# mconati/armour-dev

Measured on AMD Instinct MI355X. Metric: planning iterations/sec (7-DOF, 100 t-steps, 20 obs), higher is better.
Workload: dtype f64; 1 GPU; Kinova Gen3 7-DOF, T=100, O=20 box obstacles, 3 concurrent planner(s) x 1308 worlds/GPU/step; obstacles=20, worlds_per_gpu=3924, planners_per_gpu=3, worlds_per_planner=1308, parallelism=world-sharded x1, RCCL all_gather of per-world records

## Files before the change

armour-dev_amd/armour_amd/__init__.py:

```python
from __future__ import annotations

import ctypes
import os

import numpy as np

from .robots import KINOVA
from .worlds import csv_world, example_world, make_world, straight_line_waypoint

_HERE = os.path.dirname(os.path.abspath(__file__))
LIB_PATH = os.environ.get("ARMOUR_LIB") or os.path.join(_HERE, "libarmour_hip.so")
NF = 7
_LIB = None
_dp = ctypes.POINTER(ctypes.c_double)


ARMOUR_E_ARG, ARMOUR_E_HIP, ARMOUR_E_CAPACITY, ARMOUR_E_STATE, ARMOUR_E_INTERNAL = -1, -2, -3, -4, -5


class ArmourError(RuntimeError):
    pass


class Config(ctypes.Structure):
    _fields_ = [("robot", ctypes.c_int), ("num_time_steps", ctypes.c_int), ("max_obstacles", ctypes.c_int),
                ("max_worlds", ctypes.c_int), ("device", ctypes.c_int), ("max_iter", ctypes.c_int)]


class World(ctypes.Structure):
    _fields_ = [("q0", ctypes.c_double * NF), ("qd0", ctypes.c_double * NF), ("qdd0", ctypes.c_double * NF),
                ("q_des", ctypes.c_double * NF), ("num_obstacles", ctypes.c_int), ("obstacles", _dp)]


_WORLD_DTYPE = np.dtype({"names": ["q0", "qd0", "qdd0", "q_des", "num_obstacles", "obstacles"],
                         "formats": [(np.float64, NF)] * 4 + [np.int32, np.uintp],
                         "offsets": [World.q0.offset, World.qd0.offset, World.qdd0.offset, World.q_des.offset,
                                     World.num_obstacles.offset, World.obstacles.offset],
                         "itemsize": ctypes.sizeof(World)})


class ArmtdWorld(ctypes.Structure):
    _fields_ = [("q0", ctypes.c_double * NF), ("qd0", ctypes.c_double * NF), ("q_des", ctypes.c_double * NF),
                ("jrs_tables", _dp), ("k_range", ctypes.c_double * NF), ("num_obstacles", ctypes.c_int),
                ("obstacles", _dp)]


class Result(ctypes.Structure):
    _fields_ = [("k_opt", ctypes.c_double * NF), ("feasible", ctypes.c_int), ("solver_status", ctypes.c_int),
                ("iterations", ctypes.c_int), ("evaluations", ctypes.c_int), ("cost", ctypes.c_double),
                ("kkt_error", ctypes.c_double), ("error", ctypes.c_int)]


class Timing(ctypes.Structure):
    _fields_ = [("reach_ms", ctypes.c_double), ("nlp_ms", ctypes.c_double), ("total_ms", ctypes.c_double),
                ("reach_kernel_ms", ctypes.c_double), ("reach_bytes", ctypes.c_double)]

    def as_dict(self):
        return {name: getattr(self, name) for name, _ in self._fields_}


class PlanOutput(ctypes.Structure):
    _fields_ = [("result", Result), ("timing", Timing), ("constraints", _dp), ("joint_bounds", _dp),
                ("link_centers", _dp), ("link_generators", _dp), ("torque_radius", _dp)]


def lib():
    global _LIB
    if _LIB is None:
        if not os.path.exists(LIB_PATH):
            raise ArmourError(f"HIP planner library not built: {LIB_PATH} (run __graft_entry__.build())")
        L = ctypes.CDLL(LIB_PATH)
        L.armour_create.restype = ctypes.c_void_p
        L.armour_create.argtypes = [ctypes.POINTER(Config)]
        L.armour_create_robot.restype = ctypes.c_void_p
        L.armour_create_robot.argtypes = [ctypes.POINTER(Config), ctypes.c_void_p]
        L.armour_robot_builtin.argtypes = [ctypes.c_int, ctypes.c_void_p]
        L.armour_device_compute_units.argtypes = [ctypes.c_int]
        L.armour_copy_bandwidth.restype = ctypes.c_double
        L.armour_copy_bandwidth.argtypes = [ctypes.c_int, ctypes.c_size_t, ctypes.c_int]
        L.armour_destroy.argtypes = [ctypes.c_void_p]
        L.armour_last_error.restype = ctypes.c_char_p
        L.armour_num_constraints.argtypes = [ctypes.c_void_p, ctypes.c_int]
        L.armour_num_joints.argtypes = [ctypes.c_void_p]
        L.armour_create_armtd.restype = ctypes.c_void_p
        L.armour_create_armtd.argtypes = [ctypes.POINTER(Config)]
        L.armour_plan_armtd_batch.argtypes = [ctypes.c_void_p, ctypes.c_int, ctypes.POINTER(ArmtdWorld),
                                              ctypes.POINTER(Result), ctypes.POINTER(Timing)]
        L.armour_reach_armtd_batch.argtypes = [ctypes.c_void_p, ctypes.c_int, ctypes.POINTER(ArmtdWorld),
                                               ctypes.POINTER(Timing)]
        L.armour_plan_batch.argtypes = [ctypes.c_void_p, ctypes.c_int, ctypes.POINTER(World), ctypes.POINTER(Result),
                                        ctypes.POINTER(Timing)]
        L.armour_reach_batch.argtypes = [ctypes.c_void_p, ctypes.c_int, ctypes.POINTER(World), ctypes.POINTER(Timing)]
        for name, args in (("armour_plan_batch_mixed", L.armour_plan_batch.argtypes),
                           ("armour_reach_batch_mixed", L.armour_reach_batch.argtypes),
                           ("armour_world_num_obstacles", [ctypes.c_void_p, ctypes.c_int]),
                           ("armour_eval_candidates", [ctypes.c_void_p, ctypes.c_int, _dp, _dp, _dp,
                                                       ctypes.POINTER(ctypes.c_int), ctypes.POINTER(ctypes.c_int)])):
            if hasattr(L, name):
                getattr(L, name).argtypes = args
        L.armour_plan.argtypes = [ctypes.c_void_p, ctypes.POINTER(World), ctypes.POINTER(PlanOutput)]
        L.armour_eval_constraints.argtypes = [ctypes.c_void_p, ctypes.c_int, _dp, _dp, _dp]
        L.armour_get_reach_program.argtypes = [ctypes.c_void_p, ctypes.POINTER(ctypes.c_int), ctypes.c_int]
        L.armour_get_monomial_counts.argtypes = [ctypes.c_void_p, ctypes.c_int, ctypes.POINTER(ctypes.c_int),
                                                 ctypes.POINTER(ctypes.c_int)]
        L.armour_get_reach_occupancy.argtypes = [ctypes.c_void_p, ctypes.POINTER(ctypes.c_longlong),
                                                 ctypes.POINTER(ctypes.c_longlong), ctypes.c_int]
        L.armour_get_joint_bounds.argtypes = [ctypes.c_void_p, _dp]
        L.armour_get_plane_cache_stats.argtypes = [ctypes.c_void_p, ctypes.POINTER(ctypes.c_longlong), ctypes.c_int]
        L.armour_get_reach_span.argtypes = [ctypes.c_void_p, _dp]
        L.armour_get_reach_dump.argtypes = [ctypes.c_void_p, _dp, ctypes.c_int]
        L.armour_get_reach_profile.argtypes = [ctypes.c_void_p, ctypes.POINTER(ctypes.c_ulonglong), ctypes.c_int]
        for name in ("armour_get_constraints", "armour_get_link_centers", "armour_get_link_generators",
                     "armour_get_torque_radius"):
            getattr(L, name).argtypes = [ctypes.c_void_p, ctypes.c_int, _dp]
        if hasattr(L, "armour_sq_selfcheck"):
            L.armour_sq_selfcheck.argtypes = [ctypes.c_int, ctypes.c_double, ctypes.c_longlong, _dp, ctypes.c_longlong,
                                              _dp, ctypes.POINTER(ctypes.c_int), ctypes.POINTER(ctypes.c_longlong)]
        _LIB = L
    return _LIB


ABI_SYMBOLS = ["armour_copy_bandwidth", "armour_create", "armour_create_robot", "armour_robot_builtin", "armour_device_compute_units", "armour_destroy", "armour_last_error", "armour_num_constraints",
               "armour_plan_batch", "armour_reach_batch", "armour_eval_constraints", "armour_get_constraints",
               "armour_get_link_centers", "armour_get_link_generators", "armour_get_torque_radius",
               "armour_num_joints", "armour_get_joint_bounds", "armour_get_reach_program", "armour_get_reach_profile",
               "armour_get_reach_dump", "armour_get_reach_occupancy", "armour_get_monomial_counts",
               "armour_create_armtd", "armour_plan_armtd_batch", "armour_reach_armtd_batch",
               "armour_get_plane_cache_stats", "armour_plan", "armour_get_reach_span",
               "armour_plan_batch_mixed", "armour_reach_batch_mixed", "armour_world_num_obstacles",
               "armour_eval_candidates", "armour_sq_selfcheck"]


def default_batch(T: int, device: int = 0, waves: int = 2) -> int:
    n = lib().armour_device_compute_units(device)
    _check(min(0, n))
    return max(1, (waves * n * 64) // T)


def copy_bandwidth(device: int = 0, nbytes: int = 2 << 30, reps: int = 10) -> float:
    v = lib().armour_copy_bandwidth(device, nbytes, reps)
    if v < 0:
        raise ArmourError(f"armour_copy_bandwidth: {lib().armour_last_error().decode()}")
    return v


def sq_selfcheck(thr: float, half_width: int, values=None, device: int = 0):
    v = np.ascontiguousarray(values if values is not None else np.zeros(0), dtype=np.float64)
    s, ok, bad = ctypes.c_double(0), ctypes.c_int(0), ctypes.c_longlong(0)
    _check(lib().armour_sq_selfcheck(device, float(thr), int(half_width), _ptr(v) if v.size else None, v.size,
                                     ctypes.byref(s), ctypes.byref(ok), ctypes.byref(bad)))
    return s.value, bool(ok.value), int(bad.value)


def _check(rc):
    if rc != 0:
        raise ArmourError(f"armour error {rc}: {lib().armour_last_error().decode()}")


def _ptr(a):
    return a.ctypes.data_as(_dp) if a is not None else None


def candidates_array(x, W):
    x = np.asarray(x, dtype=np.float64)
    if x.ndim == 2 and x.shape[1] == NF and x.shape[0] >= 1:
        if W < 1:
            raise ValueError("eval_candidates: x of shape [N, 7] needs a batch (reach or plan first)")
        x = np.broadcast_to(x, (W,) + x.shape)
    if x.ndim != 3 or x.shape[2] != NF or x.shape[0] < 1 or x.shape[1] < 1 or (W >= 1 and x.shape[0] != W):
        raise ValueError(f"eval_candidates: x must have shape [W, N, {NF}] or [N, {NF}] (W = {W}), got {x.shape}")
    if not np.all(np.isfinite(x)):
        raise ValueError("eval_candidates: x holds a non-finite value")
    if np.abs(x).max() > 1.0:
        raise ValueError("eval_candidates: every candidate must lie in [-1, 1]")
    return np.ascontiguousarray(x)


class Planner:

    def __init__(self, T=100, max_obstacles=20, max_worlds=1, device=0, max_iter=0, robot=None, _armtd=False):
        cfg = Config(0, T, max_obstacles, max_worlds, device, max_iter)
        if _armtd:
            self.h = lib().armour_create_armtd(ctypes.byref(cfg))
        elif robot is None:
            self.h = lib().armour_create(ctypes.byref(cfg))
        else:
            from .robot_tables import to_struct
            self._robot = to_struct(robot)
            self.h = lib().armour_create_robot(ctypes.byref(cfg), ctypes.byref(self._robot))
        if not self.h:
            raise ArmourError(f"armour_create failed: {lib().armour_last_error().decode()}")
        self.T = T
        self.NJ = lib().armour_num_joints(self.h)
        self.max_worlds = max_worlds
        self._keep = []
        self.O = 0
        self._W = 0

    def close(self):
        if getattr(self, "h", None) and _LIB is not None:
            _LIB.armour_destroy(self.h)
        self.h = None

    def __del__(self):
        self.close()

    def num_constraints(self, O):
        return lib().armour_num_constraints(self.h, O)

    def _worlds(self, worlds):
        n = len(worlds)
        arr = (World * n)()
        view = np.frombuffer(arr, dtype=_WORLD_DTYPE)
# ... 89 lines not shown
        J = np.zeros((m, NF)) if jac else None
        _check(lib().armour_eval_constraints(self.h, w, _ptr(x), _ptr(g), _ptr(J)))
        return (g, J) if jac else g

    def eval_candidates(self, x, num_worlds=None):
        x = candidates_array(x, self._W if num_worlds is None else int(num_worlds))
        Wx, N = x.shape[:2]
        cost = np.zeros((Wx, N))
        viol = np.zeros((Wx, N, 3))
        feas = np.zeros((Wx, N), dtype=np.int32)
        best = np.zeros(Wx, dtype=np.int32)
        ip = ctypes.POINTER(ctypes.c_int)
        _check(lib().armour_eval_candidates(self.h, N, _ptr(x), _ptr(cost), _ptr(viol), feas.ctypes.data_as(ip),
                                            best.ctypes.data_as(ip)))
        return dict(cost=cost, violation=viol, feasible=feas.astype(bool), best=best)

    def constraints(self, w):
        g = np.zeros(self._m(w))
        _check(lib().armour_get_constraints(self.h, w, _ptr(g)))
        return g

    def link_centers(self, w):
        c = np.zeros((self.T, self.NJ, 3))
        _check(lib().armour_get_link_centers(self.h, w, _ptr(c)))
        return c

    def link_generators(self, w):
        g = np.zeros((self.T, self.NJ, 3, 6))
        _check(lib().armour_get_link_generators(self.h, w, _ptr(g)))
        return g

    def joint_bounds(self):
        b = np.zeros(28)
        _check(lib().armour_get_joint_bounds(self.h, _ptr(b)))
        return b

    def reach_program(self):
        n = lib().armour_get_reach_program(self.h, None, 0)
        codes = (ctypes.c_int * n)()
        lib().armour_get_reach_program(self.h, codes, n)
        return np.array(codes[:])

    def reach_dump(self):
        n = lib().armour_get_reach_dump(self.h, None, 0)
        if n < 0:
            _check(n)
        d = np.zeros((n, 8))
        _check(min(0, lib().armour_get_reach_dump(self.h, _ptr(d), n)))
        return d

    def reach_profile(self):
        n = lib().armour_get_reach_profile(self.h, None, 0)
        if n < 0:
            _check(n)
        buf = (ctypes.c_ulonglong * (2 * n + 16))()
        _check(min(0, lib().armour_get_reach_profile(self.h, buf, n + 8)))
        a = np.array(buf[:], dtype=np.uint64)
        return a[:2 * n].reshape(n, 2), a[2 * n:]

    def monomial_counts(self, w):
        lk = np.zeros((self.T, self.NJ), dtype=np.int32)
        tq = np.zeros((self.T, NF), dtype=np.int32)
        _check(lib().armour_get_monomial_counts(self.h, w, lk.ctypes.data_as(ctypes.POINTER(ctypes.c_int)),
                                                tq.ctypes.data_as(ctypes.POINTER(ctypes.c_int))))
        return lk, tq

    OCCUPANCY = ("arena_hashes", "arena_rows", "operator_terms", "link_monomials", "torque_monomials",
                 "worlds_retried", "worlds_failed")

    def occupancy(self):
        n = len(self.OCCUPANCY)
        used = (ctypes.c_longlong * n)()
        caps = (ctypes.c_longlong * n)()
        rc = lib().armour_get_reach_occupancy(self.h, used, caps, n)
        _check(min(0, rc))
        return {k: (int(used[i]), int(caps[i])) for i, k in enumerate(self.OCCUPANCY)}

    def reach_span_ms(self):
        v = ctypes.c_double()
        _check(lib().armour_get_reach_span(self.h, ctypes.byref(v)))
        return v.value

    def plane_cache_stats(self):
        keys = ("planes_kept", "pairs", "blocks_cached", "blocks", "max_per_pair", "pool_records", "box_misses")
        out = (ctypes.c_longlong * len(keys))()
        _check(min(0, lib().armour_get_plane_cache_stats(self.h, out, len(keys))))
        return {k: int(out[i]) for i, k in enumerate(keys)}

    def torque_radius(self, w):
        r = np.zeros((self.T, NF))
        _check(lib().armour_get_torque_radius(self.h, w, _ptr(r)))
        return r


class ArmtdPlanner(Planner):

    def __init__(self, T=100, max_obstacles=20, max_worlds=1, device=0, max_iter=0):
        super().__init__(T=T, max_obstacles=max_obstacles, max_worlds=max_worlds, device=device, max_iter=max_iter,
                         _armtd=True)

    def _worlds(self, worlds):
        n = len(worlds)
        arr = (ArmtdWorld * n)()
        keep = []
        for k, (q0, qd0, q_des, tab, kr, obs) in enumerate(worlds):
            a = arr[k]
            a.q0[:] = [float(v) for v in q0]
            a.qd0[:] = [float(v) for v in qd0]
            a.q_des[:] = [float(v) for v in q_des]
            a.k_range[:] = [float(v) for v in kr]
            t = np.ascontiguousarray(np.asarray(tab, dtype=np.float64).reshape(NF, 6, self.T))
            o = np.ascontiguousarray(np.asarray(obs, dtype=np.float64).reshape(-1, 12))
            keep += [t, o]
            a.jrs_tables = _ptr(t)
            a.num_obstacles = o.shape[0]
            a.obstacles = _ptr(o) if o.shape[0] else None
        self._keep = keep
        self.O = arr[0].num_obstacles if n else 0
        self._W = n
        return arr

    def _plan_call(self, *a):
        return lib().armour_plan_armtd_batch(*a)

    def _reach_call(self, *a):
        return lib().armour_reach_armtd_batch(*a)


__all__ = ["ArmtdPlanner", "Planner", "ArmourError", "ARMOUR_E_CAPACITY", "ARMOUR_E_INTERNAL", "copy_bandwidth", "default_batch", "make_world", "example_world", "csv_world", "straight_line_waypoint", "KINOVA", "LIB_PATH", "ABI_SYMBOLS", "candidates_array"]
```

armour-dev_amd/csrc/nlp.h:

```cpp
#pragma once
#include "reach.h"

namespace armour {

constexpr int EVAL_THREADS = 256;
constexpr int ROW_THREADS = 256;
constexpr int MAX_FILTER = 64;
constexpr int KA = 56;
constexpr int KA2 = 8;

struct IpmOpts {
    double tol = 1e-4;
    int max_iter = 100;
    double mu0 = 0.1;
    double kappa_eps = 10.0;
    double kappa_mu = 0.2;
    double theta_mu = 1.5;
    double tau_min = 0.99;
    double bound_push = 1e-2;
    double eta = 1e-4;
    int max_ls = 10;
    double kappa_sigma = 1e10;
    double s_max = 100.0;
    double inf_bound = 1e19;
// ... 5 lines not shown
};

struct WorldState {
    double x[NF], xt[NF], dx[NF];
    double H[NF * NF];
    double mu, alpha, ap, ad, theta0, phi0, Dphi, theta_max, theta_min, kkt;
    double sw_dphi, sw_theta;
    double wa_old_a[NF], wa_old_b[NF];
    double filt_theta[MAX_FILTER], filt_phi[MAX_FILTER];
    int nfilt;
    int cur;
    int status;
    int searching;
    int accepted_ok;
    int ftype;
    int first_update, nfail, iter, nevals, ls;
    int spec_k;
    int free_mode, nref;
    double kkt_ref[4];
    int nresto, rstall, rpend;
    double rphi;
};
constexpr int WS_RESTO = 6;
constexpr int WS_RESTART = 7;

struct NlpDev {
    int W, T, NJ, O, m, R, nblk, chunk;
    int armtd, nt;
    const double* krange;
    int diag;
    const RobotParams* rp;
    IpmOpts opt;
    const double* q0;
    const double* qd0;
    const double* qdd0;
    const double* qdes;
    const double* obs;
    ReachOut ro;
    double *L, *U;
    double* g;
    double* J;
    double* jn;
    double* jd;
    long njn, njd;
    double* f;
    double* grad;
    double* link_c;
    long lcs;
    double *slo, *shi, *zlo, *zhi, *dslo, *dshi;
    double* partial;
    double* partial2;
    WorldState* ws;
    int* flags;
    const int* wl;
    int* wl_run;
    int* wl_search;
    unsigned* cnt;
    int ls0;
    const unsigned* lcount;
    unsigned* lcount_out;
    unsigned* lrun_out;
    int* nrun_flag;
    int* bt_flag;
    int K;
    double *gs, *fs, *partial_s;
    int b_in_cs;
    int resto;
    int rflag;
    int* rl_app;
    int* pend_flag;
    int pcache;
    int pcready;
    long pc_pool;
    double* pc;
    uint16_t* pcp;
    unsigned* pcoff;
    unsigned char* pcok;
    unsigned long long* pcbase;
    unsigned* pcnext;
    const int* Ow;
};
constexpr int EV_MAXK = 9;
constexpr int PC_K = 12;
constexpr double PC_XBOX = 1.0 + 1e-6;
constexpr double PC_RADF = 1.0001;
constexpr double PC_MARGIN = 1e-9;

AD int world_of(const NlpDev& d, int b) { return d.wl ? d.wl[b] : b; }

AD long gidx(const NlpDev& d, int slot, int w, long r) { return ((long)slot * d.W + w) * d.m + r; }

struct Shape {
    int O, m, R, nblk;
};
template <bool MX>
AD Shape shape_of(const NlpDev& d, int w) {
    if constexpr (MX) {
        const int O = d.Ow[w];
        const int m = d.nt + d.T * d.NJ * O + 4 * NF;
        const int R = m + NF;
        return Shape{O, m, R, (R + d.chunk - 1) / d.chunk};
    } else {
        return Shape{d.O, d.m, d.R, d.nblk};
    }
}

}
```

armour-dev_amd/csrc/nlp_kernels.hip:

```cpp
#include "nlp.h"

namespace armour {

__device__ inline double wave_max(double v) {
#pragma unroll
    for (int m = 1; m < 64; m <<= 1) v = fmax(v, xor_f64(v, m));
    return v;
}
__device__ inline double wave_min(double v) {
#pragma unroll
    for (int m = 1; m < 64; m <<= 1) v = fmin(v, xor_f64(v, m));
    return v;
}
template <int N>
__device__ inline void block_reduce_n(double (&v)[N], const int (&kinds)[N], double* lds, double* out) {
    const int wave = threadIdx.x >> 6, nw = blockDim.x >> 6;
#pragma unroll
    for (int g = 0; g < N; g += 8) {
#pragma unroll
        for (int i = g; i < (g + 8 < N ? g + 8 : N); i++)
            v[i] = kinds[i] == 0 ? wave_sum(v[i]) : kinds[i] == 1 ? wave_max(v[i]) : wave_min(v[i]);
        if ((threadIdx.x & 63) == 0) {
#pragma unroll
            for (int i = g; i < (g + 8 < N ? g + 8 : N); i++) lds[wave * N + i] = v[i];
// ... 595 lines not shown
    pw[0] = (R)1.0; pw[1] = xj; pw[2] = xj * xj; pw[3] = xj * xj * xj;
}
__device__ __attribute__((always_inline)) double value_term(double co, int h, const double (*pw)[4]) {
    double v = co;
#pragma unroll
    for (int j = 0; j < NF; j++) v = v * pw[j][(h >> (2 * j)) & 3];
    return v;
}

struct TrajStart {
    const double *q0, *qd0, *qdd0;
    double D;
};
__device__ __attribute__((always_inline)) TrajStart traj_start(const NlpDev& d, int w) {
    return {d.q0 + w * NF, d.qd0 + w * NF, d.qdd0 + w * NF, d.rp->duration};
}
struct ExtremumRows {
    double mn, mx, scale, e2, e3;
    int mnid, mxid;
};
__device__ __attribute__((always_inline)) ExtremumRows extremum_rows(const RobotParams& rp, TrajStart s, int kind,
                                                                     int j, double xj) {
    ExtremumRows r;
    double mn, mx;
    extremum(kind, s.q0[j], s.qd0[j] * s.D, s.qdd0[j] * s.D * s.D, rp.k_range[j] * xj, &mn, &mx, &r.mnid, &r.mxid, &r.e2, &r.e3);
    r.scale = kind == 0 ? 1.0 : s.D;
    r.mn = mn / r.scale;
    r.mx = mx / r.scale;
    return r;
}
#define TRAJ_COST_BODY                                                                              \
    for (int j = 0; j < NF; j++)                                                                    \
        qp[j] = bz_q(ts.q0[j], ts.qd0[j] * ts.D, ts.qdd0[j] * ts.D * ts.D, rp.k_range[j] * x[j], tp); \
    double fv = 0.0;                                                                                \
    bool first = true;                                                                              \
    for (int pass = 1; pass >= 0; pass--)                                                           \
        for (int j = 0; j < NF; j++) {                                                              \
            if (rp.wrap_mask[j] != pass) continue;                                                  \
            const double dd = pass ? wrap_to_pi(d.qdes[w * NF + j] - qp[j]) : (d.qdes[w * NF + j] - qp[j]); \
            const double term = dd * dd;                                                            \
            fv = first ? term : fv + term;                                                          \
            first = false;                                                                          \
        }
__device__ __attribute__((always_inline)) double traj_cost(const NlpDev& d, const RobotParams& rp, TrajStart ts, int w,
                                                           const double* x, double* qp) {
    const double tp = rp.t_plan;
    TRAJ_COST_BODY
    return fv;
}

struct PlaneRecords {
    const double* rec;
    const uint16_t* pcp;
    int total;
};
__device__ __attribute__((always_inline)) PlaneRecords plane_records(const NlpDev& d, long jt, int NP, bool some = true) {
    const unsigned last = some ? d.pcoff[jt * (d.NJ * d.O) + NP - 1] : 0u;
    const unsigned long long pb = d.pcbase[jt];
    return {d.pc + 5 * pb, d.pcp + pb, (int)(last >> 8) + (int)(last & 255)};
}
struct PlaneRecord {
    double a[3], P, N;
    int pr;
};
__device__ __attribute__((always_inline)) PlaneRecord load_record(PlaneRecords pc, int q) {
    const int cap = pc.total;
    return {{pc.rec[q], pc.rec[cap + q], pc.rec[2 * cap + q]}, pc.rec[3 * cap + q], pc.rec[4 * cap + q], pc.pcp[q]};
}
__device__ __attribute__((always_inline)) double record_candidate(PlaneRecord r, const double* lc, bool& neg) {
    const double Ac = r.a[0] * lc[0] + r.a[1] * lc[1] + r.a[2] * lc[2];
    const double pos = Ac - r.P, nv = -Ac - r.N;
    neg = nv > pos || pos != pos;
    return neg ? nv : pos;
}
constexpr double SCAN_START = -100000000.0;
__device__ __attribute__((always_inline)) void pair_max(unsigned long long* key, double v) {
    if (v > SCAN_START) atomicMax(key, okey(v));
}

constexpr int UB_FULL = MAX_J * CAP_LM * 3 + NF * CAP_UM;
constexpr int LM_S = 16, UM_S = 64;
constexpr int UB_S = 1544;
static_assert(UB_S >= MAX_J * LM_S * 3 + NF * UM_S, "small staging buffer");
__host__ __device__ constexpr int eval_pair_doubles(int np) { return np + (np + 1) / 2 + 4 * np; }
template <typename R, bool ARMTD, bool CACHED, int LM, int UM, int UB, bool MX = false>
__device__ __attribute__((always_inline)) void eval_body(const NlpDev& d, int mode) {
    static_assert(!CACHED || std::is_same<R, double>::value, "the plane cache is fp64");
    static_assert(!MX || (std::is_same<R, double>::value && !ARMTD), "mixed batches: the fp64 ARMOUR planner");
    if ((mode == 1 || mode == 5) && d.lcount && blockIdx.y >= *d.lcount) return;
    const int t = blockIdx.x, w = world_of(d, blockIdx.y);
    WorldState& S = d.ws[w];
    if (mode == 1 && !((d.resto ? S.status == WS_RESTO : S.status == 0) && S.searching)) return;
    if (mode == 5 && !(d.resto ? (S.status == WS_RESTO && S.rpend) : (S.status == 0 && S.spec_k >= 0))) return;
    EVP_DECL EVP_MARK
    const int slot = mode == 0 ? 0 : 1 - S.cur;
    double* const Gb = d.g + gidx(d, slot, w, 0);
    double* const Jb = d.J + gidx(d, slot, w, 0) * NF;
    double* const Lcb = d.link_c + slot * d.lcs + (long)w * d.T * d.NJ * 3;
    double* const fb = d.f + slot * d.W + w;
    double* const gradb = d.grad + ((long)slot * d.W + w) * NF;
    const long ncol = (long)d.T * d.NJ * d.O;
    double* const Jnb = d.jn + slot * d.njn + (long)w * ncol * 3;
    double* const Jdb = d.jd + slot * d.njd + (long)w * d.T * d.NJ * NF * 3;
    const RobotParams& rp = *d.rp;
    const int tid = threadIdx.x;
    const long jt = (long)w * d.T + t;
    const int NJ = d.NJ, O = shape_of<MX>(d, w).O, OS = d.O;
    __shared__ double x[NF];
    __shared__ R lc[MAX_J][3];
    __shared__ R dlc[MAX_J][NF][3];
    __shared__ R lgen[MAX_J][18];
    __shared__ R obs[MAX_OBS][12];
    __shared__ uint16_t lh[MAX_J][LM];
    __shared__ uint16_t th[NF][UM];
    __shared__ double ubuf[UB];
    static_assert(MAX_J * LM * 3 + NF * UM <= UB, "monomial staging");
    auto lco = reinterpret_cast<R (*)[LM][3]>(ubuf);
    auto tco = reinterpret_cast<R (*)[UM]>(ubuf + MAX_J * LM * 3);
    constexpr int NMIX = MAX_J * MAX_OBS * OBS_GEN;
    static_assert(CACHED || MAX_J * LL_PLANES * 10 + MAX_OBS * OO_PLANES * 5 + NMIX + (NMIX + 7) / 8 <= UB, "plane tables");
    auto llp = reinterpret_cast<R (*)[LL_PLANES][10]>(ubuf);
    auto oop = reinterpret_cast<R (*)[OO_PLANES][5]>(ubuf + MAX_J * LL_PLANES * 10);
    R* mixv = reinterpret_cast<R*>(ubuf + MAX_J * LL_PLANES * 10 + MAX_OBS * OO_PLANES * 5);
    int8_t* mixc = reinterpret_cast<int8_t*>(mixv + NMIX);
    __shared__ int lcnt[MAX_J], tcnt[NF];
    __shared__ R ptab[NF][8];
    if (tid < NF) {
        const double xd = mode == 0 ? S.x[tid] : S.xt[tid];
        x[tid] = xd;
        const R xj = (R)xd;
        power_table(xj, ptab[tid]);
        ptab[tid][4] = (R)0.0; ptab[tid][5] = (R)1.0 * (R)1.0; ptab[tid][6] = (R)2.0 * xj; ptab[tid][7] = (R)3.0 * (xj * xj);
    }
    if (tid < NJ) lcnt[tid] = d.ro.link_cnt[jt * NJ + tid];
    if (tid >= 32 && tid < 32 + NF) tcnt[tid - 32] = d.nt ? d.ro.tq_cnt[jt * NF + tid - 32] : 0;
    if constexpr (!CACHED) {
        for (int i = tid; i < NJ * 18; i += blockDim.x) lgen[i / 18][i % 18] = d.ro.link_gens[jt * NJ * 18 + i];
        for (int i = tid; i < O * 12; i += blockDim.x) obs[i / 12][i % 12] = d.obs[(long)w * OS * 12 + i];
    }
    __syncthreads();
    EVP_MARK
    if (!(d.diag & 1)) {
        STAGE_MONOMIALS_BODY
    }
    __syncthreads();
    EVP_MARK
    const int nlk = NJ * 3 * 8;
    for (int u = tid; u < ((d.diag & 1) ? 0 : 64 + nlk); u += blockDim.x) {
      if (u >= 64) {
        const int ul = u - 64;
        const int l = ul / 24, e = (ul / 8) % 3, k = ul % 8;
        const long base = jt * NJ + l;
        R c = k == 0 ? d.ro.link_center[base * 3 + e] : 0.0;
        c = sum4(c, lcnt[l], [&](int q) { return slice_term(lco[l][q][e], lh[l][q], k, ptab); });
        if (k == 0) {
            const R r = d.ro.link_rad[base * 3 + e];
            const R cc = interval_mid(c, r);
            lc[l][e] = cc;
            Lcb[((long)t * NJ + l) * 3 + e] = cc;
        } else {
            dlc[l][k - 1][e] = c;
            Jdb[(((long)t * NJ + l) * NF + k - 1) * 3 + e] = c;
        }
      } else {
        if (u >= NF * 8 || d.nt == 0) continue;
        const int j = u / 8, k = u % 8;
        const long base = jt * NF + j;
        R c = k == 0 ? d.ro.tq_center[base] : 0.0;
        c = sum4(c, tcnt[j], [&](int q) { return slice_term(tco[j][q], th[j][q], k, ptab); });
        const long gi = (long)t * NF + j;
        if (k == 0) {
            const R r = d.ro.tq_rad[base];
            Gb[gi] = interval_mid(c, r);
        } else {
            Jb[gi * NF + k - 1] = c;
        }
      }
    }
    if constexpr (ARMTD) {
        if (tid == blockDim.x - 1 && t == 0) armtd_extrema_cost(d, w, x, Gb, Jb, fb, gradb);
    } else if (t == 0 && tid >= (int)blockDim.x - 2 * NF - 1) {
        const TrajStart ts = traj_start(d, w);
        const int v = tid - ((int)blockDim.x - 2 * NF - 1);
        if (v < 2 * NF) {
            const long off2 = (long)NF * d.T + (long)d.T * d.NJ * O;
            const int kind = v / NF, i = v % NF;
            const ExtremumRows er = extremum_rows(rp, ts, kind, i, x[i]);
            const long gmin = off2 + kind * 2 * NF + i, gmax = gmin + NF;
            Gb[gmin] = er.mn;
            Gb[gmax] = er.mx;
            const double gmn = extremum_grad(kind, er.mnid, er.e2, er.e3) * rp.k_range[i] / er.scale;
            const double gmx = extremum_grad(kind, er.mxid, er.e2, er.e3) * rp.k_range[i] / er.scale;
#pragma unroll
            for (int k = 0; k < NF; k++) {
                Jb[gmin * NF + k] = (k == i) ? gmn : 0.0;
                Jb[gmax * NF + k] = (k == i) ? gmx : 0.0;
            }
        } else {
            const double tp = rp.t_plan;
            double qp[NF];
            TRAJ_COST_BODY
            *fb = fv * rp.cost_scale;
            for (int i = 0; i < NF; i++) {
                const double dk = tp * tp * tp * (6 * tp * tp - 15 * tp + 10) * rp.k_range[i];
                double gv = rp.wrap_mask[i] ? (2 * wrap_to_pi(qp[i] - d.qdes[w * NF + i]) * dk) : (2 * (qp[i] - d.qdes[w * NF + i]) * dk);
                gradb[i] = gv * rp.cost_scale;
            }
        }
    }
    __syncthreads();
    EVP_MARK
    const long nt = d.nt;
    bool coll = !(d.diag & 2);
    if constexpr (MX) coll = coll && O > 0;
    if constexpr (CACHED) {
        bool inbox = true;
#pragma unroll
        for (int j = 0; j < NF; j++) inbox = inbox && fabs(x[j]) <= PC_XBOX;
        if (coll && !inbox) {
            for (int pr = tid; pr < NJ * O; pr += blockDim.x)
                Gb[nt + ((long)(pr / O) * d.T + t) * O + pr % O] = __builtin_nan("");
            if (tid == 0) atomicAdd(d.cnt + 7, 1u);
        } else if (coll) {
            const int NP = NJ * O;
            const PlaneRecords pc = plane_records(d, jt, NP);
            const int total = pc.total;
            unsigned long long* const pkey = reinterpret_cast<unsigned long long*>(ubuf);
            unsigned* const pidx = reinterpret_cast<unsigned*>(ubuf + NP);
            double* const pB = ubuf + NP + (NP + 1) / 2;
            static_assert(eval_pair_doubles(MAX_J * MAX_OBS) <= UB_FULL, "pair tables");
            const double start = SCAN_START;
            for (int pr = tid; pr < NP; pr += blockDim.x) {
                pkey[pr] = okey(start);
                pidx[pr] = 0xFFFFFFFFu;
            }
            __syncthreads();
            EVP_MARK
            auto cand = [&](int q, double& v, int& sub, int& pr, double* a) {
                const PlaneRecord r = load_record(pc, q);
                a[0] = r.a[0]; a[1] = r.a[1]; a[2] = r.a[2];
                pr = r.pr;
                bool neg;
                v = record_candidate(r, lc[pr / O], neg);
                sub = neg ? 1 : 0;
            };
            constexpr int RPT = 3;
            if (total <= RPT * EVAL_THREADS) {
                double v[RPT], a[RPT][3];
                int sub[RPT], pq[RPT];
#pragma unroll
                for (int s = 0; s < RPT; s++) {
                    const int q = tid + s * EVAL_THREADS;
                    v[s] = start;
                    sub[s] = 0;
                    pq[s] = 0;
                    if (q < total) {
                        cand(q, v[s], sub[s], pq[s], a[s]);
                        pair_max(&pkey[pq[s]], v[s]);
                    }
                }
                __syncthreads();
                EVP_MARK
#pragma unroll
                for (int s = 0; s < RPT; s++) {
                    const int q = tid + s * EVAL_THREADS;
                    if (q < total && v[s] > start && v[s] == dkey(pkey[pq[s]])) atomicMin(&pidx[pq[s]], (unsigned)(2 * q + sub[s]));
                }
                __syncthreads();
                EVP_MARK
#pragma unroll
                for (int s = 0; s < RPT; s++) {
                    const int q = tid + s * EVAL_THREADS;
                    if (q < total && pidx[pq[s]] == (unsigned)(2 * q + sub[s])) {
                        double* const b = pB + pq[s] * 4;
                        b[0] = a[s][0]; b[1] = a[s][1]; b[2] = a[s][2]; b[3] = v[s];
                    }
                }
            } else {
                for (int q = tid; q < total; q += blockDim.x) {
                    double v, a[3];
                    int sub, pr;
                    cand(q, v, sub, pr, a);
                    pair_max(&pkey[pr], v);
                }
                __syncthreads();
                EVP_MARK
                for (int q = tid; q < total; q += blockDim.x) {
                    double v, a[3];
                    int sub, pr;
                    cand(q, v, sub, pr, a);
                    if (v > start && v == dkey(pkey[pr])) atomicMin(&pidx[pr], (unsigned)(2 * q + sub));
                }
                __syncthreads();
                EVP_MARK
                for (int q = tid; q < total; q += blockDim.x) {
                    double v, a[3];
                    int sub, pr;
                    cand(q, v, sub, pr, a);
                    if (pidx[pr] == (unsigned)(2 * q + sub)) {
                        double* const b = pB + pr * 4;
                        b[0] = a[0]; b[1] = a[1]; b[2] = a[2]; b[3] = v;
                    }
                }
            }
            __syncthreads();
            EVP_MARK
            for (int pr = tid; pr < NP; pr += blockDim.x) {
                const int l = pr / O, o = pr % O;
                const unsigned wi = pidx[pr];
                const bool won = wi != 0xFFFFFFFFu, isneg = won && (wi & 1u);
                const double* const b = pB + pr * 4;
                const double best = won ? b[3] : start;
                const double B0 = won ? b[0] : 0.0, B1 = won ? b[1] : 0.0, B2 = won ? b[2] : 0.0;
                const long row = nt + ((long)l * d.T + t) * O + o;
                Gb[row] = -best;
                double* const jn = Jnb + (row - nt) * 3;
                jn[0] = isneg ? B0 : -B0;
                jn[1] = isneg ? B1 : -B1;
                jn[2] = isneg ? B2 : -B2;
                if (mode == 0) {
#pragma unroll
                    for (int kk = 0; kk < NF; kk++) {
                        const double dot = B0 * dlc[l][kk][0] + B1 * dlc[l][kk][1] + B2 * dlc[l][kk][2];
                        Jb[row * NF + kk] = isneg ? dot : -dot;
                    }
                }
            }
            coll = false;
        }
    }
    if constexpr (!CACHED) {
    for (int u = tid; u < (coll ? NJ * LL_PLANES + O * OO_PLANES : 0); u += blockDim.x) {
        if (u < NJ * LL_PLANES) {
            const int l = u / LL_PLANES, p = u % LL_PLANES;
            ll_table(lgen[l], p, lc[l], llp[l][p]);
        } else {
            const int v = u - NJ * LL_PLANES, o = v / OO_PLANES, p = v % OO_PLANES;
            oo_table(obs[o], p, oop[o][p]);
        }
    }
    const int nmix = coll ? NJ * O * OBS_GEN : 0;
    for (int u = tid; u < nmix; u += blockDim.x) {
        const int l = u / (O * OBS_GEN), o = (u / OBS_GEN) % O, i = u % OBS_GEN;
        const R c0 = lc[l][0], c1 = lc[l][1], c2 = lc[l][2];
        R G[BUF_GEN][3], oc[3];
#pragma unroll
        for (int r = 0; r < 3; r++) oc[r] = obs[o][r];
#pragma unroll
        for (int q = 0; q < OBS_GEN; q++)
#pragma unroll
            for (int r = 0; r < 3; r++) G[q][r] = obs[o][(q + 1) * 3 + r];
#pragma unroll
        for (int q = 0; q < 6; q++)
#pragma unroll
            for (int r = 0; r < 3; r++) G[OBS_GEN + q][r] = lgen[l][r + 3 * q];
        R ga[3];
#pragma unroll
        for (int r = 0; r < 3; r++) ga[r] = obs[o][(i + 1) * 3 + r];
        const R cc[3] = {c0, c1, c2};
        R best = -100000000.0;
        int code = -1;
        auto scan = [&](auto e_tag, int j) {
            constexpr int E = decltype(e_tag)::value;
            R A[3], dd, del;
            mixed_plane<E>(ga, G[OBS_GEN + j], G, oc, A, dd, del);
            const R Ac = dot_z<E>(A, cc);
            if (A[0] != 0 || A[1] != 0 || A[2] != 0) {
                const R pos = Ac - (dd + del);
                const R neg = -Ac - (-dd + del);
                if (pos > best) { best = pos; code = 2 * j; }
                if (neg > best) { best = neg; code = 2 * j + 1; }
            }
        };
        using gen = std::integral_constant<int, -1>;
        scan(gen{}, 0);
        scan(gen{}, 1);
        scan(gen{}, 2);
        scan(std::integral_constant<int, 0>{}, 3);
        scan(std::integral_constant<int, 1>{}, 4);
        scan(std::integral_constant<int, 2>{}, 5);
        mixv[u] = best;
        mixc[u] = (int8_t)code;
    }
    __syncthreads();
    EVP_MARK
    for (int pr = tid; pr < (coll ? NJ * O : 0); pr += blockDim.x) {
        const int l = pr / O, o = pr % O;
        R best = -100000000.0;
        R B0 = 0, B1 = 0, B2 = 0;
        bool isneg = false;
        int mwin = -1;
        const R c0 = lc[l][0], c1 = lc[l][1], c2 = lc[l][2];
        R G[BUF_GEN][3], oc[3];
#pragma unroll
        for (int r = 0; r < 3; r++) oc[r] = obs[o][r];
#pragma unroll
// ... 1749 lines not shown
```

armour-dev_amd/csrc/planner.hip:

```cpp
#include <hip/hip_runtime.h>
#include <chrono>
#include <cstdio>
#include <cstdlib>
#include <cstring>
#include <algorithm>
#include <atomic>
#include <string>
#include <vector>

#include "../../include/armour_hip.h"
#include "nlp_kernels.hip"
#include "reach_kernel.hip"
#include "lane_kernel.hip"
#include "robots.h"

using namespace armour;

namespace {
thread_local std::string g_err;

int fail(int code, const std::string& msg) {
    g_err = msg;
    return code;
}
// ... 1548 lines not shown
    HIPCK(hipMemcpy(radius, p->ro.torque_radius + (size_t)w * p->T * NF, sizeof(double) * p->T * NF, hipMemcpyDeviceToHost));
    return 0;
}

int armour_get_reach_profile(armour_planner* p, unsigned long long* cycles_terms, int capacity) {
    DeviceScope device_scope(p);
    if (!p) return fail(ARMOUR_E_ARG, "null planner");
    if (!p->d_prof) return fail(ARMOUR_E_STATE, "op profiling is off (set ARMOUR_PROFILE_OPS before armour_create)");
    if (cycles_terms && capacity >= p->nops + 8) {
        const size_t nb = ((size_t)p->Wmax * p->T + lane::LG - 1) / lane::LG;
        const size_t n = capacity >= p->nops + 8 + 4 * OP_NCODES + (long)nb ? 2 * p->nops + 16 + 8 * OP_NCODES + 2 * nb
                         : capacity >= p->nops + 8 + 4 * OP_NCODES ? 2 * p->nops + 16 + 8 * OP_NCODES : 2 * p->nops + 16;
        HIPCK(hipMemcpy(cycles_terms, p->d_prof, sizeof(unsigned long long) * n, hipMemcpyDeviceToHost));
    }
    return p->nops;
}

int armour_get_reach_dump(armour_planner* p, double* dump, int capacity) {
    DeviceScope device_scope(p);
    if (!p) return fail(ARMOUR_E_ARG, "null planner");
    if (!p->d_dump) return fail(ARMOUR_E_STATE, "op dump is off (set ARMOUR_DUMP_OPS before armour_create)");
    if (!p->lane_engine && p->has_lane)
        return fail(ARMOUR_E_STATE, "the op dump follows the bundle engine, and the last batch ran on the per-job engine");
    if (dump && capacity >= p->nops) {
        if (p->lane_engine) {
            const char* ls = std::getenv("ARMOUR_DUMP_LANE");
            const int l = ls ? std::atoi(ls) & 63 : 0;
            std::vector<double> all((size_t)p->nops * DUMP_W * lane::LG);
            HIPCK(hipMemcpy(all.data(), p->d_dump, sizeof(double) * all.size(), hipMemcpyDeviceToHost));
            for (int k = 0; k < p->nops * DUMP_W; k++) dump[k] = all[(size_t)k * lane::LG + l];
        } else {
            HIPCK(hipMemcpy(dump, p->d_dump, sizeof(double) * DUMP_W * p->nops, hipMemcpyDeviceToHost));
        }
    }
    return p->nops;
}

int armour_get_monomial_counts(armour_planner* p, int w, int* link_counts, int* torque_counts) {
    DeviceScope device_scope(p);
    if (!p) return fail(ARMOUR_E_ARG, "null planner");
    if (!p->reached) return fail(ARMOUR_E_STATE, "no reach set");
    if (w < 0 || w >= p->W) return fail(ARMOUR_E_ARG, "world index out of range");
    const size_t j0 = (size_t)w * p->T;
    if (link_counts)
        HIPCK(hipMemcpy(link_counts, p->ro.link_cnt + j0 * p->NJ, sizeof(int) * p->T * p->NJ, hipMemcpyDeviceToHost));
    if (torque_counts)
        HIPCK(hipMemcpy(torque_counts, p->ro.tq_cnt + j0 * NF, sizeof(int) * p->T * NF, hipMemcpyDeviceToHost));
    return 0;
}

int armour_get_reach_span(armour_planner* p, double* span_ms) {
    if (!p || !span_ms) return fail(ARMOUR_E_ARG, "null planner or output");
    if (!p->reached) return fail(ARMOUR_E_STATE, "no reach set");
    *span_ms = p->last_span_ms;
    return p->last_span_ms >= 0 ? 0 : fail(ARMOUR_E_STATE, "no device clock span for the last reach");
}

int armour_get_plane_cache_stats(armour_planner* p, long long* out, int n) {
    DeviceScope device_scope(p);
    if (!p) return fail(ARMOUR_E_ARG, "null planner");
    if (!p->reached) return fail(ARMOUR_E_STATE, "no reach set");
    NlpDev& d = p->d;
    if (!d.pcache || p->eval_f32 || d.O == 0) return fail(ARMOUR_E_STATE, "plane cache off (ARMOUR_PLANE_CACHE=0, float study or no obstacles)");
    ensure_plane_cache(p);
    const size_t blocks = (size_t)p->W * p->T, NP = (size_t)p->NJ * d.O;
    std::vector<unsigned> off(blocks * NP);
    std::vector<unsigned char> ok(blocks);
    HIPCK(hipMemcpyAsync(off.data(), d.pcoff, sizeof(unsigned) * off.size(), hipMemcpyDeviceToHost, p->stream));
    HIPCK(hipMemcpyAsync(ok.data(), d.pcok, blocks, hipMemcpyDeviceToHost, p->stream));
    HIPCK(hipStreamSynchronize(p->stream));
    long long kept = 0, nok = 0, mx = 0, pairs = 0;
    for (size_t b = 0; b < blocks; b++) {
        const size_t np = (size_t)p->NJ * p->Ow[b / p->T];
        pairs += (long long)np;
        for (size_t q = 0; q < np; q++) {
            const unsigned v = off[b * NP + q];
            kept += v & 255;
            mx = std::max<long long>(mx, v & 255);
        }
    }
    for (unsigned char v : ok) nok += v;
    unsigned miss = 0;
    HIPCK(hipMemcpy(&miss, d.cnt + 7, sizeof(unsigned), hipMemcpyDeviceToHost));
    const long long st[ARMOUR_PC_COUNT] = {kept, pairs, nok, (long long)blocks, mx, d.pc_pool, miss};
    for (int k = 0; k < n && k < ARMOUR_PC_COUNT; k++) out[k] = st[k];
    return ARMOUR_PC_COUNT;
}

int armour_get_reach_occupancy(armour_planner* p, long long* used, long long* caps, int n) {
    DeviceScope device_scope(p);
    if (!p) return fail(ARMOUR_E_ARG, "null planner");
    if (!p->reached) return fail(ARMOUR_E_STATE, "no reach set");
    if (!p->lane_engine || !p->d_occ)
        return fail(ARMOUR_E_STATE, "occupancy is recorded by the bundle engine only (this batch ran on the per-job engine)");
    const unsigned long long* o = p->h_occ;
    const long long u[ARMOUR_OCC_COUNT] = {(long long)o[0], (long long)o[1], (long long)o[2], (long long)o[3],
                                           (long long)o[4], p->last_retried, p->last_failed};
    const long long c[ARMOUR_OCC_COUNT] = {p->la.hcap, p->la.ccap, std::min<long long>(p->la.gcap, (1 << 16) - 1),
                                           CAP_LM, CAP_UM, p->W, p->W};
    for (int k = 0; k < n && k < ARMOUR_OCC_COUNT; k++) {
        if (used) used[k] = u[k];
        if (caps) caps[k] = c[k];
    }
    return ARMOUR_OCC_COUNT;
}

int armour_get_reach_program(const armour_planner* p, int* codes, int capacity) {
    DeviceScope device_scope(p);
    if (!p) return fail(ARMOUR_E_ARG, "null planner");
    if (codes && capacity >= p->nops) {
        std::vector<Op> ops(p->nops);
        HIPCK(hipMemcpy(ops.data(), p->d_prog, sizeof(Op) * p->nops, hipMemcpyDeviceToHost));
        for (int k = 0; k < p->nops; k++) codes[k] = ops[k].code;
    }
    return p->nops;
}

}
```

include/armour_hip.h:

```cpp
#ifndef ARMOUR_HIP_H
#define ARMOUR_HIP_H

#include <stddef.h>

#ifdef __cplusplus
extern "C" {
#endif

#define ARMOUR_NUM_FACTORS 7
#define ARMOUR_OBSTACLE_DOUBLES 12

enum {
    ARMOUR_OK = 0,
    ARMOUR_E_ARG = -1,
    ARMOUR_E_HIP = -2,
    ARMOUR_E_CAPACITY = -3,
    ARMOUR_E_STATE = -4,
    ARMOUR_E_INTERNAL = -5
};

typedef struct armour_planner armour_planner;

typedef struct armour_config {
    int robot;
// ... 37 lines not shown

#define ARMOUR_MAX_JOINTS 9
typedef struct armour_robot {
    int num_joints;
    int axes[ARMOUR_MAX_JOINTS];
    int wrap[ARMOUR_NUM_FACTORS];
    double trans[(ARMOUR_MAX_JOINTS + 1) * 3];
    double rots[ARMOUR_MAX_JOINTS * 3];
    double mass[ARMOUR_MAX_JOINTS];
    double com[ARMOUR_MAX_JOINTS * 3];
    double inertia[ARMOUR_MAX_JOINTS * 9];
    double mass_uncertainty, inertia_uncertainty;
    double friction[ARMOUR_MAX_JOINTS], damping[ARMOUR_MAX_JOINTS], armature[ARMOUR_MAX_JOINTS];
    double state_lb[ARMOUR_NUM_FACTORS], state_ub[ARMOUR_NUM_FACTORS];
    double speed_limits[ARMOUR_NUM_FACTORS], torque_limits[ARMOUR_NUM_FACTORS];
    double gravity;
    double link_center[ARMOUR_MAX_JOINTS * 3], link_generators[ARMOUR_MAX_JOINTS * 3];
    double alpha, V_m, M_max, M_min, K;
} armour_robot;

int armour_device_compute_units(int device);

double armour_copy_bandwidth(int device, size_t bytes, int reps);

int armour_robot_builtin(int robot_id, armour_robot* out);
armour_planner* armour_create_robot(const armour_config* cfg, const armour_robot* robot);
const char* armour_last_error(void);

int armour_num_constraints(const armour_planner* p, int num_obstacles);

int armour_plan_batch(armour_planner* p, int num_worlds, const armour_world* worlds, armour_result* results,
                      armour_timing* timing);

int armour_plan_batch_mixed(armour_planner* p, int num_worlds, const armour_world* worlds, armour_result* results,
                            armour_timing* timing);
int armour_reach_batch_mixed(armour_planner* p, int num_worlds, const armour_world* worlds, armour_timing* timing);
int armour_world_num_obstacles(const armour_planner* p, int w);

typedef struct armour_plan_output {
    armour_result result;
    armour_timing timing;
    double* constraints;
    double* joint_bounds;
    double* link_centers;
    double* link_generators;
    double* torque_radius;
} armour_plan_output;
int armour_plan(armour_planner* p, const armour_world* world, armour_plan_output* out);

typedef struct armour_armtd_world {
    double q0[ARMOUR_NUM_FACTORS];
    double qd0[ARMOUR_NUM_FACTORS];
    double q_des[ARMOUR_NUM_FACTORS];
    const double* jrs_tables;
    double k_range[ARMOUR_NUM_FACTORS];
    int num_obstacles;
    const double* obstacles;
} armour_armtd_world;

armour_planner* armour_create_armtd(const armour_config* cfg);
int armour_plan_armtd_batch(armour_planner* p, int num_worlds, const armour_armtd_world* worlds,
                            armour_result* results, armour_timing* timing);
int armour_reach_armtd_batch(armour_planner* p, int num_worlds, const armour_armtd_world* worlds, armour_timing* timing);

int armour_reach_batch(armour_planner* p, int num_worlds, const armour_world* worlds, armour_timing* timing);

int armour_eval_constraints(armour_planner* p, int w, const double* x, double* g, double* jac);

int armour_eval_candidates(armour_planner* p, int num_candidates, const double* x, double* cost, double* violation,
                           int* feasible, int* best);

int armour_get_constraints(armour_planner* p, int w, double* g);
int armour_get_link_centers(armour_planner* p, int w, double* centers);
int armour_get_link_generators(armour_planner* p, int w, double* gens);
int armour_get_torque_radius(armour_planner* p, int w, double* radius);
int armour_num_joints(const armour_planner* p);
int armour_get_monomial_counts(armour_planner* p, int w, int* link_counts, int* torque_counts);
int armour_get_joint_bounds(const armour_planner* p, double* bounds28);

int armour_get_reach_program(const armour_planner* p, int* codes, int capacity);
#define ARMOUR_OCC_COUNT 7
int armour_get_reach_occupancy(armour_planner* p, long long* used, long long* caps, int n);
int armour_get_reach_profile(armour_planner* p, unsigned long long* cycles_terms, int capacity);
#define ARMOUR_PC_COUNT 7
int armour_get_plane_cache_stats(armour_planner* p, long long* out, int n);
int armour_get_reach_span(armour_planner* p, double* span_ms);
int armour_get_reach_dump(armour_planner* p, double* dump, int capacity);
int armour_sq_selfcheck(int device, double thr, long long half_width, const double* values, long long n,
                        double* s_star, int* valid, long long* mismatches);

#ifdef __cplusplus
}
#endif
#endif
```

Baseline: 6956 plans/s.

## Hold more plane-cache candidates in registers and drop the pair staging table

The plane-cache eval kernel used to handle up to 3 records per thread in registers, with a three-pass fallback that reloaded records. It now keeps up to EVAL_RPT (default 8) records per thread in registers, packs the pair index and sign into one word, and streams any overflow records. The third pass that copied the winning plane into a shared table is removed; the winner record is reloaded once per pair in the write-out loop, which cuts shared memory and a barrier. The trade-off is higher register pressure from the larger unrolled arrays, which may lower occupancy. A diagnostic API that reports per-block record counts is also added.

```diff
diff --git a/armour-dev_amd/armour_amd/__init__.py b/armour-dev_amd/armour_amd/__init__.py
--- a/armour-dev_amd/armour_amd/__init__.py
+++ b/armour-dev_amd/armour_amd/__init__.py
@@ -94,6 +94,8 @@
         for name, args in (("armour_plan_batch_mixed", L.armour_plan_batch.argtypes),
                            ("armour_reach_batch_mixed", L.armour_reach_batch.argtypes),
                            ("armour_world_num_obstacles", [ctypes.c_void_p, ctypes.c_int]),
+                           ("armour_get_plane_cache_block_records", [ctypes.c_void_p, ctypes.POINTER(ctypes.c_uint),
+                                                                     ctypes.c_longlong]),
                            ("armour_eval_candidates", [ctypes.c_void_p, ctypes.c_int, _dp, _dp, _dp,
                                                        ctypes.POINTER(ctypes.c_int), ctypes.POINTER(ctypes.c_int)])):
             if hasattr(L, name):
@@ -128,7 +130,7 @@
                "armour_create_armtd", "armour_plan_armtd_batch", "armour_reach_armtd_batch",
                "armour_get_plane_cache_stats", "armour_plan", "armour_get_reach_span",
                "armour_plan_batch_mixed", "armour_reach_batch_mixed", "armour_world_num_obstacles",
-               "armour_eval_candidates", "armour_sq_selfcheck"]
+               "armour_eval_candidates", "armour_sq_selfcheck", "armour_get_plane_cache_block_records"]
 
 
 def default_batch(T: int, device: int = 0, waves: int = 2) -> int:
@@ -384,10 +386,18 @@
         return v.value
 
     def plane_cache_stats(self):
-        keys = ("planes_kept", "pairs", "blocks_cached", "blocks", "max_per_pair", "pool_records", "box_misses")
+        keys = ("planes_kept", "pairs", "blocks_cached", "blocks", "max_per_pair", "pool_records", "box_misses",
+                "register_records")
         out = (ctypes.c_longlong * len(keys))()
         _check(min(0, lib().armour_get_plane_cache_stats(self.h, out, len(keys))))
         return {k: int(out[i]) for i, k in enumerate(keys)}
+
+    def plane_cache_block_records(self):
+        n = lib().armour_get_plane_cache_block_records(self.h, None, 0)
+        _check(min(0, n))
+        out = np.zeros(n, dtype=np.uint32)
+        _check(min(0, lib().armour_get_plane_cache_block_records(self.h, out.ctypes.data_as(ctypes.POINTER(ctypes.c_uint)), n)))
+        return out.reshape(-1, self.T)
 
     def torque_radius(self, w):
         r = np.zeros((self.T, NF))
diff --git a/armour-dev_amd/csrc/nlp.h b/armour-dev_amd/csrc/nlp.h
--- a/armour-dev_amd/csrc/nlp.h
+++ b/armour-dev_amd/csrc/nlp.h
@@ -111,6 +111,10 @@
 };
 constexpr int EV_MAXK = 9;
 constexpr int PC_K = 12;
+#ifndef EVAL_RPT
+#define EVAL_RPT 8
+#endif
+__host__ __device__ constexpr int eval_register_records(int diag) { return ((diag & 4) ? 1 : EVAL_RPT) * EVAL_THREADS; }
 constexpr double PC_XBOX = 1.0 + 1e-6;
 constexpr double PC_RADF = 1.0001;
 constexpr double PC_MARGIN = 1e-9;
diff --git a/armour-dev_amd/csrc/nlp_kernels.hip b/armour-dev_amd/csrc/nlp_kernels.hip
--- a/armour-dev_amd/csrc/nlp_kernels.hip
+++ b/armour-dev_amd/csrc/nlp_kernels.hip
@@ -701,7 +701,8 @@
 constexpr int LM_S = 16, UM_S = 64;
 constexpr int UB_S = 1544;
 static_assert(UB_S >= MAX_J * LM_S * 3 + NF * UM_S, "small staging buffer");
-__host__ __device__ constexpr int eval_pair_doubles(int np) { return np + (np + 1) / 2 + 4 * np; }
+__host__ __device__ constexpr int eval_pair_doubles(int np) { return np + (np + 1) / 2; }
+static_assert(eval_pair_doubles(MAX_J * MAX_OBS) <= UB_S, "pair tables (small)");
 template <typename R, bool ARMTD, bool CACHED, int LM, int UM, int UB, bool MX = false>
 __device__ __attribute__((always_inline)) void eval_body(const NlpDev& d, int mode) {
     static_assert(!CACHED || std::is_same<R, double>::value, "the plane cache is fp64");
@@ -846,8 +847,8 @@
             const int total = pc.total;
             unsigned long long* const pkey = reinterpret_cast<unsigned long long*>(ubuf);
             unsigned* const pidx = reinterpret_cast<unsigned*>(ubuf + NP);
-            double* const pB = ubuf + NP + (NP + 1) / 2;
             static_assert(eval_pair_doubles(MAX_J * MAX_OBS) <= UB_FULL, "pair tables");
+            static_assert(MAX_J * MAX_OBS < (1 << 15), "pair and sign in one word");
             const double start = SCAN_START;
             for (int pr = tid; pr < NP; pr += blockDim.x) {
                 pkey[pr] = okey(start);
@@ -855,72 +856,46 @@
             }
             __syncthreads();
             EVP_MARK
-            auto cand = [&](int q, double& v, int& sub, int& pr, double* a) {
+            auto cand = [&](int q, double& v) {
                 const PlaneRecord r = load_record(pc, q);
-                a[0] = r.a[0]; a[1] = r.a[1]; a[2] = r.a[2];
-                pr = r.pr;
                 bool neg;
-                v = record_candidate(r, lc[pr / O], neg);
-                sub = neg ? 1 : 0;
+                v = record_candidate(r, lc[r.pr / O], neg);
+                return (unsigned)r.pr | (neg ? 0x8000u : 0u);
             };
-            constexpr int RPT = 3;
-            if (total <= RPT * EVAL_THREADS) {
-                double v[RPT], a[RPT][3];
-                int sub[RPT], pq[RPT];
-#pragma unroll
-                for (int s = 0; s < RPT; s++) {
+            const int nreg = min(total, eval_register_records(d.diag));
+            double v[EVAL_RPT];
+            unsigned ps[EVAL_RPT];
+#pragma unroll
+            for (int s = 0; s < EVAL_RPT; s++) {
+                v[s] = start;
+                ps[s] = 0;
+                if (s * EVAL_THREADS < nreg) {
                     const int q = tid + s * EVAL_THREADS;
-                    v[s] = start;
-                    sub[s] = 0;
-                    pq[s] = 0;
-                    if (q < total) {
-                        cand(q, v[s], sub[s], pq[s], a[s]);
-                        pair_max(&pkey[pq[s]], v[s]);
+                    if (q < nreg) {
+                        ps[s] = cand(q, v[s]);
+                        pair_max(&pkey[ps[s] & 0x7FFFu], v[s]);
                     }
                 }
-                __syncthreads();
-                EVP_MARK
-#pragma unroll
-                for (int s = 0; s < RPT; s++) {
+            }
+            for (int q = nreg + tid; q < total; q += EVAL_THREADS) {
+                double vq;
+                const unsigned p = cand(q, vq);
+                pair_max(&pkey[p & 0x7FFFu], vq);
+            }
+            __syncthreads();
+            EVP_MARK
+#pragma unroll
+            for (int s = 0; s < EVAL_RPT; s++) {
+                if (s * EVAL_THREADS < nreg) {
                     const int q = tid + s * EVAL_THREADS;
-                    if (q < total && v[s] > start && v[s] == dkey(pkey[pq[s]])) atomicMin(&pidx[pq[s]], (unsigned)(2 * q + sub[s]));
+                    const unsigned pr = ps[s] & 0x7FFFu;
+                    if (q < nreg && v[s] > start && v[s] == dkey(pkey[pr])) atomicMin(&pidx[pr], (unsigned)(2 * q) + (ps[s] >> 15));
                 }
-                __syncthreads();
-                EVP_MARK
-#pragma unroll
-                for (int s = 0; s < RPT; s++) {
-                    const int q = tid + s * EVAL_THREADS;
-                    if (q < total && pidx[pq[s]] == (unsigned)(2 * q + sub[s])) {
-                        double* const b = pB + pq[s] * 4;
-                        b[0] = a[s][0]; b[1] = a[s][1]; b[2] = a[s][2]; b[3] = v[s];
-                    }
-                }
-            } else {
-                for (int q = tid; q < total; q += blockDim.x) {
-                    double v, a[3];
-                    int sub, pr;
-                    cand(q, v, sub, pr, a);
-                    pair_max(&pkey[pr], v);
-                }
-                __syncthreads();
-                EVP_MARK
-                for (int q = tid; q < total; q += blockDim.x) {
-                    double v, a[3];
-                    int sub, pr;
-                    cand(q, v, sub, pr, a);
-                    if (v > start && v == dkey(pkey[pr])) atomicMin(&pidx[pr], (unsigned)(2 * q + sub));
-                }
-                __syncthreads();
-                EVP_MARK
-                for (int q = tid; q < total; q += blockDim.x) {
-                    double v, a[3];
-                    int sub, pr;
-                    cand(q, v, sub, pr, a);
-                    if (pidx[pr] == (unsigned)(2 * q + sub)) {
-                        double* const b = pB + pr * 4;
-                        b[0] = a[0]; b[1] = a[1]; b[2] = a[2]; b[3] = v;
-                    }
-                }
+            }
+            for (int q = nreg + tid; q < total; q += EVAL_THREADS) {
+                double vq;
+                const unsigned p = cand(q, vq), pr = p & 0x7FFFu;
+                if (vq > start && vq == dkey(pkey[pr])) atomicMin(&pidx[pr], (unsigned)(2 * q) + (p >> 15));
             }
             __syncthreads();
             EVP_MARK
@@ -928,9 +903,13 @@
                 const int l = pr / O, o = pr % O;
                 const unsigned wi = pidx[pr];
                 const bool won = wi != 0xFFFFFFFFu, isneg = won && (wi & 1u);
-                const double* const b = pB + pr * 4;
-                const double best = won ? b[3] : start;
-                const double B0 = won ? b[0] : 0.0, B1 = won ? b[1] : 0.0, B2 = won ? b[2] : 0.0;
+                double best = start, B0 = 0.0, B1 = 0.0, B2 = 0.0;
+                if (won) {
+                    const PlaneRecord r = load_record(pc, (int)(wi >> 1));
+                    bool neg;
+                    best = record_candidate(r, lc[l], neg);
+                    B0 = r.a[0]; B1 = r.a[1]; B2 = r.a[2];
+                }
                 const long row = nt + ((long)l * d.T + t) * O + o;
                 Gb[row] = -best;
                 double* const jn = Jnb + (row - nt) * 3;
diff --git a/armour-dev_amd/csrc/planner.hip b/armour-dev_amd/csrc/planner.hip
--- a/armour-dev_amd/csrc/planner.hip
+++ b/armour-dev_amd/csrc/planner.hip
@@ -1654,9 +1654,29 @@
     for (unsigned char v : ok) nok += v;
     unsigned miss = 0;
     HIPCK(hipMemcpy(&miss, d.cnt + 7, sizeof(unsigned), hipMemcpyDeviceToHost));
-    const long long st[ARMOUR_PC_COUNT] = {kept, pairs, nok, (long long)blocks, mx, d.pc_pool, miss};
+    const long long st[ARMOUR_PC_COUNT] = {kept, pairs, nok, (long long)blocks, mx, d.pc_pool, miss,
+                                           eval_register_records(d.diag)};
     for (int k = 0; k < n && k < ARMOUR_PC_COUNT; k++) out[k] = st[k];
     return ARMOUR_PC_COUNT;
+}
+
+int armour_get_plane_cache_block_records(armour_planner* p, unsigned* out, long long n) {
+    DeviceScope device_scope(p);
+    if (!p) return fail(ARMOUR_E_ARG, "null planner");
+    if (!p->reached) return fail(ARMOUR_E_STATE, "no reach set");
+    NlpDev& d = p->d;
+    if (!d.pcache || p->eval_f32 || d.O == 0) return fail(ARMOUR_E_STATE, "plane cache off (ARMOUR_PLANE_CACHE=0, float study or no obstacles)");
+    ensure_plane_cache(p);
+    const size_t blocks = (size_t)p->W * p->T, NP = (size_t)p->NJ * d.O;
+    std::vector<unsigned> off(blocks * NP);
+    HIPCK(hipMemcpyAsync(off.data(), d.pcoff, sizeof(unsigned) * off.size(), hipMemcpyDeviceToHost, p->stream));
+    HIPCK(hipStreamSynchronize(p->stream));
+    for (size_t b = 0; b < blocks && (long long)b < n; b++) {
+        const size_t np = (size_t)p->NJ * p->Ow[b / p->T];
+        const unsigned last = np ? off[b * NP + np - 1] : 0u;
+        out[b] = (last >> 8) + (last & 255);
+    }
+    return (int)blocks;
 }
 
 int armour_get_reach_occupancy(armour_planner* p, long long* used, long long* caps, int n) {
diff --git a/include/armour_hip.h b/include/armour_hip.h
--- a/include/armour_hip.h
+++ b/include/armour_hip.h
@@ -143,8 +143,9 @@
 #define ARMOUR_OCC_COUNT 7
 int armour_get_reach_occupancy(armour_planner* p, long long* used, long long* caps, int n);
 int armour_get_reach_profile(armour_planner* p, unsigned long long* cycles_terms, int capacity);
-#define ARMOUR_PC_COUNT 7
+#define ARMOUR_PC_COUNT 8
 int armour_get_plane_cache_stats(armour_planner* p, long long* out, int n);
+int armour_get_plane_cache_block_records(armour_planner* p, unsigned* out, long long n);
 int armour_get_reach_span(armour_planner* p, double* span_ms);
 int armour_get_reach_dump(armour_planner* p, double* dump, int capacity);
 int armour_sq_selfcheck(int device, double thr, long long half_width, const double* values, long long n,
```

After: 7045 plans/s (median of 6 runs). No clear change (+1.3%).
